# THUDM/CogDL

Measured on NVIDIA B200. Metric: spmm_aggregated_edges_per_sec, higher is better.
Workload: dtype f32

## Files before the change

cogdl_b200/csrc/common.cuh:

```cuda
#pragma once
#include <cuda_runtime.h>
#include <stdint.h>

#include "../../include/cogdl_b200.h"

#if defined(__CUDA_ARCH__) && (__CUDA_ARCH__ < 1000)
#error "libcogdl_b200 is written for sm_100a (B200) only"
#endif

namespace cogdl_b200 {

int set_error(int code, const char *fmt, ...);
void count_launch(int n = 1);
void note_kernel(const char *fmt, ...);
void append_kernel_note(const char *fmt, ...);
int tuning(const char *env_name, int dflt);

#define CB_REQUIRE(cond, ...)                                             \
  do {                                                                    \
    if (!(cond)) return ::cogdl_b200::set_error(COGDL_B200_EINVAL, __VA_ARGS__); \
  } while (0)

#define CB_CUDA(expr)                                                                       \
  do {                                                                                      \
    cudaError_t _e = (expr);                                                                \
    if (_e != cudaSuccess)                                                                  \
      return ::cogdl_b200::set_error(_e == cudaErrorNoKernelImageForDevice ? COGDL_B200_EDEVICE \
                                                                           : COGDL_B200_ECUDA, \
                                     "%s: %s", #expr, cudaGetErrorString(_e));              \
  } while (0)

#define CB_LAUNCH_CHECK()                  \
  do {                                     \
    ::cogdl_b200::count_launch();          \
    CB_CUDA(cudaPeekAtLastError());        \
  } while (0)

static inline bool first_use_on_device(unsigned long long &mask, int *dev) {
  *dev = 0;
  if (cudaGetDevice(dev) != cudaSuccess || *dev < 0 || *dev >= 64) return true;
  const unsigned long long bit = 1ull << *dev;
  if (mask & bit) return false;
  mask |= bit;
  return true;
}

static inline bool aligned16(const void *p) { return (reinterpret_cast<uintptr_t>(p) & 15u) == 0; }
static inline int64_t ceil_div(int64_t a, int64_t b) { return (a + b - 1) / b; }

struct HubView {
  int chunk_edges;
  int n_chunks;
  const int2 *chunks;
  int *counters;
  void *partials;
  int n_segs;
  const int2 *segs;
  const int *edge_row;
  int n_empty_rows;
};

static inline HubView hub_view(const cogdl_b200_hub_plan_t *plan) {
  HubView h{0, 0, nullptr, nullptr, nullptr, 0, nullptr, nullptr, 0};
  if (plan && plan->chunk_edges > 0) {
    h.chunk_edges = plan->chunk_edges;
    h.n_chunks = plan->n_chunks;
    h.chunks = reinterpret_cast<const int2 *>(plan->chunks);
    h.counters = plan->counters;
    h.partials = plan->partials;
    if (plan->segs && plan->edge_row && plan->n_segs > 0) {
      h.n_segs = plan->n_segs;
      h.segs = reinterpret_cast<const int2 *>(plan->segs);
      h.edge_row = plan->edge_row;
      h.n_empty_rows = plan->n_empty_rows;
    }
  }
  return h;
}

int check_plan(const cogdl_b200_hub_plan_t *plan, int64_t need_partial_bytes);

#ifdef __CUDACC__

constexpr unsigned FULL = 0xffffffffu;

__device__ __forceinline__ int ld_stream(const int *p) {
  int v;
  asm volatile("ld.global.nc.L1::no_allocate.s32 %0, [%1];" : "=r"(v) : "l"(p));
  return v;
}
__device__ __forceinline__ float ld_stream(const float *p) {
  float v;
  asm volatile("ld.global.nc.L1::no_allocate.f32 %0, [%1];" : "=f"(v) : "l"(p));
  return v;
}
__device__ __forceinline__ float4 ld_gather(const float4 *p) { return __ldg(p); }
__device__ __forceinline__ float ld_gather(const float *p) { return __ldg(p); }

__device__ __forceinline__ uint64_t l2_policy_evict_last() {
  uint64_t pol;
  asm volatile("createpolicy.fractional.L2::evict_last.b64 %0, 1.0;" : "=l"(pol));
  return pol;
}
__device__ __forceinline__ float4 ld_gather_hint(const float4 *p, uint64_t pol) {
  float4 v;
  asm volatile("ld.global.nc.L2::cache_hint.v4.f32 {%0,%1,%2,%3}, [%4], %5;"
               : "=f"(v.x), "=f"(v.y), "=f"(v.z), "=f"(v.w) : "l"(p), "l"(pol));
  return v;
}
__device__ __forceinline__ float ld_gather_hint(const float *p, uint64_t pol) {
  float v;
  asm volatile("ld.global.nc.L2::cache_hint.f32 %0, [%1], %2;" : "=f"(v) : "l"(p), "l"(pol));
  return v;
}

__device__ __forceinline__ void st_stream(float4 *p, float4 v) { __stcs(p, v); }
__device__ __forceinline__ void st_stream(float *p, float v) { __stcs(p, v); }
__device__ __forceinline__ void st_stream(int *p, int v) { __stcs(p, v); }

__device__ __forceinline__ float4 ld_cg(const float4 *p) { return __ldcg(p); }
__device__ __forceinline__ float ld_cg(const float *p) { return __ldcg(p); }
__device__ __forceinline__ int ld_cg(const int *p) { return __ldcg(p); }
__device__ __forceinline__ void st_cg(float4 *p, float4 v) { __stcg(p, v); }
__device__ __forceinline__ void st_cg(float *p, float v) { __stcg(p, v); }
__device__ __forceinline__ void st_cg(int *p, int v) { __stcg(p, v); }

__device__ __forceinline__ float mul_add_rn(float acc, float v, float x) {
  return __fadd_rn(acc, __fmul_rn(v, x));
}
__device__ __forceinline__ void axpy_rn(float &acc, float v, const float &x) { acc = mul_add_rn(acc, v, x); }
__device__ __forceinline__ void axpy_rn(float4 &acc, float v, const float4 &x) {
  acc.x = mul_add_rn(acc.x, v, x.x);
  acc.y = mul_add_rn(acc.y, v, x.y);
  acc.z = mul_add_rn(acc.z, v, x.z);
  acc.w = mul_add_rn(acc.w, v, x.w);
}
__device__ __forceinline__ void add_rn(float4 &acc, const float4 &x) {
  acc.x = __fadd_rn(acc.x, x.x);
  acc.y = __fadd_rn(acc.y, x.y);
  acc.z = __fadd_rn(acc.z, x.z);
  acc.w = __fadd_rn(acc.w, x.w);
}

template <int WIDTH>
__device__ __forceinline__ int group_max(int v) {
#pragma unroll
  for (int s = WIDTH / 2; s > 0; s >>= 1) v = max(v, __shfl_xor_sync(FULL, v, s));
  return v;
}
__device__ __forceinline__ int warp_max(int v) { return group_max<32>(v); }

struct WorkItem {
  int row;
  int lb, hb;
  int slot;
  int first;
  int n_row_chunks;
  bool active;
  bool is_chunk;
};

__device__ __forceinline__ WorkItem decode_item(int64_t item, int64_t n_rows, const int *__restrict__ rowptr,
                                                const HubView &hub) {
  WorkItem w;
  w.row = 0; w.lb = 0; w.hb = 0; w.slot = 0; w.first = 0; w.n_row_chunks = 0;
  w.active = false; w.is_chunk = false;
  if (item < hub.n_chunks) {
    const int2 c = __ldg(hub.chunks + item);
    const int rb = __ldg(rowptr + c.x), re = __ldg(rowptr + c.x + 1);
    w.row = c.x;
    w.first = c.y;
    w.slot = (int)item;
    w.lb = rb + ((int)item - c.y) * hub.chunk_edges;
    w.hb = min(w.lb + hub.chunk_edges, re);
    w.n_row_chunks = (re - rb + hub.chunk_edges - 1) / hub.chunk_edges;
    w.active = true;
    w.is_chunk = true;
  } else if (item - hub.n_chunks < n_rows) {
    w.row = (int)(item - hub.n_chunks);
    w.lb = __ldg(rowptr + w.row);
    w.hb = __ldg(rowptr + w.row + 1);
    w.active = !(hub.chunk_edges > 0 && (w.hb - w.lb) > hub.chunk_edges);
    if (!w.active) w.hb = w.lb;
  }
  return w;
}

template <int GROUP>
__device__ __forceinline__ bool hub_arrive_last(const WorkItem &w, const HubView &hub, int gl) {
  __threadfence();
  __syncwarp();
  int old = 0;
  if (w.is_chunk && gl == 0) old = atomicAdd(hub.counters + w.first, 1);
  old = __shfl_sync(FULL, old, 0, GROUP);
  const bool last = w.is_chunk && (old == w.n_row_chunks - 1);
  if (last) {
    if (gl == 0) hub.counters[w.first] = 0;
    __threadfence();
  }
  return last;
}

#endif

}
```

cogdl_b200/csrc/spmm.cu:

```cuda
#include "common.cuh"
#include "stream.cuh"

#include <cuda_fp16.h>

#include <cstdlib>

namespace cogdl_b200 {

struct SpmmParams {
  const float *peers[8];
  int n_peers;
  int peer_shift;
  const int *rowptr;
  const int *colind;
  const float *val;
  const float *X0;
  const float *X1;
  int64_t n0;
  float *Y;
  int64_t n_rows;
  int FV;
  HubView hub;
};

template <typename VecT> __device__ __forceinline__ VecT vzero();
template <> __device__ __forceinline__ float4 vzero<float4>() { return make_float4(0.f, 0.f, 0.f, 0.f); }
template <> __device__ __forceinline__ float vzero<float>() { return 0.f; }
__device__ __forceinline__ void add_rn(float &a, const float &b) { a = __fadd_rn(a, b); }

template <typename VecT, int GROUP, int NV, bool HAS_VAL>
__global__ void __launch_bounds__(256) spmm_kernel(const SpmmParams p) {
  constexpr int U0 = (NV == 1) ? 8 : (NV == 2 ? 4 : 2);
  constexpr int U = U0 < GROUP ? U0 : GROUP;
  constexpr int TILE = GROUP * NV;
  const int lane = threadIdx.x & 31;
  const int gl = lane & (GROUP - 1);
  const int64_t tid = (int64_t)blockIdx.x * blockDim.x + threadIdx.x;
  const int64_t item = tid / GROUP;
  const WorkItem w = decode_item(item, p.n_rows, p.rowptr, p.hub);
  const bool warp_has_chunk = (tid - lane) / GROUP < p.hub.n_chunks;

  const VecT *X0 = reinterpret_cast<const VecT *>(p.X0);
  const VecT *X1 = reinterpret_cast<const VecT *>(p.X1);
  VecT *Y = reinterpret_cast<VecT *>(p.Y);
  VecT *P = reinterpret_cast<VecT *>(p.hub.partials);

  int maxdeg = w.hb - w.lb;
  if (GROUP < 32) maxdeg = warp_max(maxdeg);

  for (int tile0 = 0; tile0 < p.FV; tile0 += TILE) {
    const int cv = tile0 + gl;
    bool colok[NV];
#pragma unroll
    for (int k = 0; k < NV; ++k) colok[k] = (cv + k * GROUP) < p.FV;
    VecT acc[NV];
#pragma unroll
    for (int k = 0; k < NV; ++k) acc[k] = vzero<VecT>();

    int c = 0;
    float v = 0.f;
    {
      const int e = w.lb + gl;
      if (e < w.hb) {
        c = ld_stream(p.colind + e);
        v = HAS_VAL ? ld_stream(p.val + e) : 1.f;
      }
    }
    for (int off = 0; off < maxdeg; off += GROUP) {
      const int cnt = min(GROUP, w.hb - w.lb - off);
      int cn = 0;
      float vn = 0.f;
      {
        const int e = w.lb + off + GROUP + gl;
        if (e < w.hb) {
          cn = ld_stream(p.colind + e);
          vn = HAS_VAL ? ld_stream(p.val + e) : 1.f;
        }
      }
#pragma unroll 1
      for (int j = 0; j < GROUP; j += U) {
        if (GROUP == 32) {
          if (j >= cnt) break;
        } else {
          if (!__any_sync(FULL, j < cnt)) break;
        }
        VecT x[U][NV];
#pragma unroll
        for (int u = 0; u < U; ++u) {
          const int cj = __shfl_sync(FULL, c, j + u, GROUP);
          if (j + u < cnt) {
            const VecT *xp = (cj < p.n0) ? X0 + (int64_t)cj * p.FV : X1 + ((int64_t)cj - p.n0) * p.FV;
#pragma unroll
            for (int k = 0; k < NV; ++k)
              if (colok[k]) x[u][k] = ld_gather(xp + cv + k * GROUP);
          }
        }
#pragma unroll
        for (int u = 0; u < U; ++u) {
          const float vj = __shfl_sync(FULL, v, j + u, GROUP);
          if (j + u < cnt) {
#pragma unroll
            for (int k = 0; k < NV; ++k)
              if (colok[k]) axpy_rn(acc[k], vj, x[u][k]);
          }
        }
      }
      c = cn;
      v = vn;
    }

    if (!w.is_chunk) {
      if (w.active) {
        VecT *yp = Y + (int64_t)w.row * p.FV + cv;
#pragma unroll
        for (int k = 0; k < NV; ++k)
          if (colok[k]) st_stream(yp + k * GROUP, acc[k]);
      }
    } else {
      VecT *pp = P + (int64_t)w.slot * p.FV + cv;
#pragma unroll
      for (int k = 0; k < NV; ++k)
        if (colok[k]) st_cg(pp + k * GROUP, acc[k]);
    }
  }

  if (warp_has_chunk) {
    if (hub_arrive_last<GROUP>(w, p.hub, gl)) {
      for (int cv = gl; cv < p.FV; cv += GROUP) {
        const VecT *pp = P + (int64_t)w.first * p.FV + cv;
        VecT s = ld_cg(pp);
        for (int q = 1; q < w.n_row_chunks; ++q) add_rn(s, ld_cg(pp + (int64_t)q * p.FV));
        st_stream(Y + (int64_t)w.row * p.FV + cv, s);
      }
    }
  }
}

static int spmm_variant() { return tuning("COGDL_B200_SPMM_VARIANT", 7); }

static StreamParams to_stream(const SpmmParams &p) {
  StreamParams q;
  q.rowptr = p.rowptr; q.colind = p.colind; q.val = p.val; q.att = nullptr; q.perm = nullptr;
  q.X0 = p.X0; q.X1 = p.X1; q.n0 = p.n0; q.Y = p.Y; q.ldv = p.FV; q.H = 1; q.FVL = p.FV; q.S = 1;
  q.hub = p.hub;
  q.n_peers = p.n_peers; q.peer_shift = p.peer_shift;
  for (int i = 0; i < 8; ++i) q.peers[i] = p.peers[i];
  return q;
}

template <typename VecT, int NV>
static int launch_spmm_stream(const SpmmParams &p, cudaStream_t stream) {
  const StreamParams q = to_stream(p);
  const int mode = p.val ? MODE_WEIGHTED : MODE_UNWEIGHTED;
  if constexpr (NV == 1 && sizeof(VecT) == 16) {
    switch (spmm_variant()) {
      case 1: return launch_stream<VecT, 1, 8, 4, false>(q, mode, stream);
      case 2: return launch_stream<VecT, 1, 8, 3, false>(q, mode, stream);
      case 3: return launch_stream<VecT, 1, 4, 6, false>(q, mode, stream);
      case 8: return launch_stream<VecT, 1, 4, 5, false, true>(q, mode, stream);
      default: return launch_stream<VecT, 1, 4, 5, false>(q, mode, stream);
    }
  }
  constexpr int U = (NV == 1) ? 8 : (NV == 2 ? 4 : 2);
  return launch_stream<VecT, NV, U, 1>(q, mode, stream);
}

template <typename VecT, int GROUP, int NV>
static int launch_spmm(const SpmmParams &p, cudaStream_t stream) {
  const int64_t items = (int64_t)p.hub.n_chunks + p.n_rows;
  const int64_t threads = items * GROUP;
  const int64_t blocks = ceil_div(threads, 256);
  if (blocks == 0) return COGDL_B200_OK;
  if (blocks > 0x7fffffffLL)
    return set_error(COGDL_B200_EINVAL, "spmm: problem too large for one launch (blocks=%lld)", (long long)blocks);
  dim3 grid((unsigned)blocks);
  note_kernel("cogdl_b200::spmm_kernel<%s,GROUP=%d,NV=%d,%s>", sizeof(VecT) == 16 ? "float4" : "float", GROUP, NV,
              p.val ? "weighted" : "unweighted");
  if (p.val)
    spmm_kernel<VecT, GROUP, NV, true><<<grid, 256, 0, stream>>>(p);
  else
    spmm_kernel<VecT, GROUP, NV, false><<<grid, 256, 0, stream>>>(p);
  CB_LAUNCH_CHECK();
  return COGDL_B200_OK;
}

template <typename VecT>
static int dispatch_spmm(const SpmmParams &p, cudaStream_t s) {
  const int fv = p.FV;
  if (p.n_peers > 0 && fv <= 32) return launch_spmm_stream<VecT, 1>(p, s);
  const bool stream = p.hub.n_segs > 0;
  const int stream_min_fv = tuning("COGDL_B200_SPMM_STREAM_MINFV", 9);
  if (stream && fv >= stream_min_fv && fv <= 16) return launch_spmm_stream<VecT, 1>(p, s);
  if (fv <= 1) return launch_spmm<VecT, 1, 1>(p, s);
  if (fv <= 2) return launch_spmm<VecT, 2, 1>(p, s);
  if (fv <= 4) return launch_spmm<VecT, 4, 1>(p, s);
  if (fv <= 8) return launch_spmm<VecT, 8, 1>(p, s);
  if (fv <= 16) return launch_spmm<VecT, 16, 1>(p, s);
  if (fv <= 32) return stream ? launch_spmm_stream<VecT, 1>(p, s) : launch_spmm<VecT, 32, 1>(p, s);
  if (sizeof(VecT) == 4 && fv > 64) return stream ? launch_spmm_stream<VecT, 4>(p, s) : launch_spmm<VecT, 32, 4>(p, s);
  return stream ? launch_spmm_stream<VecT, 2>(p, s) : launch_spmm<VecT, 32, 2>(p, s);
}

static int spmm_entry(const int32_t *rowptr, const int32_t *colind, const float *val, const float *X0,
                      int64_t n0, const float *X1, float *Y, int64_t n_rows, int64_t F,
                      const cogdl_b200_hub_plan_t *plan, cogdl_b200_stream_t stream, const char *who,
                      const float *const *peers = nullptr, int n_peers = 0, int peer_shift = 0) {
  CB_REQUIRE(n_rows >= 0 && F >= 0, "%s: negative size (n_rows=%lld, F=%lld)", who, (long long)n_rows, (long long)F);
  if (n_rows == 0 || F == 0) return COGDL_B200_OK;
  CB_REQUIRE(rowptr && colind && X0 && Y, "%s: null pointer", who);
  CB_REQUIRE(n_rows < 0x7fffffffLL && F < 0x7fffffffLL, "%s: n_rows / F must fit int32", who);
  int rc = check_plan(plan, (plan ? (int64_t)plan->n_chunks : 0) * F * (int64_t)sizeof(float));
  if (rc) return rc;
  SpmmParams p;
  p.rowptr = rowptr; p.colind = colind; p.val = val; p.X0 = X0; p.X1 = X1 ? X1 : X0; p.n0 = n0;
  p.Y = Y; p.n_rows = n_rows; p.hub = hub_view(plan);
  p.n_peers = n_peers; p.peer_shift = peer_shift;
  bool peers_aligned = true;
  for (int i = 0; i < 8; ++i) {
    p.peers[i] = (i < n_peers) ? peers[i] : nullptr;
    peers_aligned = peers_aligned && aligned16(p.peers[i]);
  }
  if (n_peers > 0)
    CB_REQUIRE(p.hub.n_segs > 0 && F % 4 == 0 && F <= 512 && peers_aligned && aligned16(X0) && aligned16(Y),
               "%s: the peer form needs a plan with segments, F %% 4 == 0, F <= 512 and 16-byte aligned buffers", who);
  const bool vec = (F % 4 == 0) && aligned16(X0) && aligned16(p.X1) && aligned16(Y) &&
                   (p.hub.n_chunks == 0 || aligned16(p.hub.partials));
  if (vec) {
    p.FV = (int)(F / 4);
    return dispatch_spmm<float4>(p, (cudaStream_t)stream);
  }
  p.FV = (int)F;
  return dispatch_spmm<float>(p, (cudaStream_t)stream);
}

struct SpmmHalfParams {
  const int *rowptr;
  const int *colind;
  const __half *val;
  const __half *X;
  __half *Y;
  int64_t n_rows;
  int F;
  HubView hub;
};

template <bool HAS_VAL, bool VEC>
__global__ void __launch_bounds__(256) spmm_half_kernel(const SpmmHalfParams p) {
  constexpr int U = 8;
  constexpr int W = VEC ? 4 : 1;
  const int lane = threadIdx.x & 31;
  const int64_t tid = (int64_t)blockIdx.x * blockDim.x + threadIdx.x;
  const WorkItem w = decode_item(tid / 32, p.n_rows, p.rowptr, p.hub);
  float *P = reinterpret_cast<float *>(p.hub.partials);

  for (int tile0 = 0; tile0 < p.F; tile0 += 32 * W) {
    const int col = tile0 + lane * W;
    const bool colok = col < p.F;
    float acc[W];
#pragma unroll
    for (int t = 0; t < W; ++t) acc[t] = 0.f;

    for (int base = w.lb; base < w.hb; base += 32) {
      const int cnt = min(32, w.hb - base);
      int c = 0;
      float v = 0.f;
      if (base + lane < w.hb) {
        c = ld_stream(p.colind + base + lane);
        v = HAS_VAL ? __half2float(p.val[base + lane]) : 1.f;
      }
#pragma unroll 1
      for (int j = 0; j < cnt; j += U) {
        float x[U][W];
#pragma unroll
        for (int u = 0; u < U; ++u) {
          const int cj = __shfl_sync(FULL, c, j + u);
          if (j + u < cnt && colok) {
            const __half *xp = p.X + (int64_t)cj * p.F + col;
            if constexpr (VEC) {
              const uint2 raw = __ldg(reinterpret_cast<const uint2 *>(xp));
              const float2 a = __half22float2(*reinterpret_cast<const __half2 *>(&raw.x));
              const float2 b = __half22float2(*reinterpret_cast<const __half2 *>(&raw.y));
              x[u][0] = a.x; x[u][1] = a.y; x[u][2] = b.x; x[u][3] = b.y;
            } else {
              x[u][0] = __half2float(__ldg(xp));
            }
          }
        }
#pragma unroll
        for (int u = 0; u < U; ++u) {
          const float vj = __shfl_sync(FULL, v, j + u);
          if (j + u < cnt && colok) {
#pragma unroll
            for (int t = 0; t < W; ++t) acc[t] = fmaf(vj, x[u][t], acc[t]);
          }
        }
      }
    }
    if (!w.is_chunk) {
      if (w.active && colok) {
        __half *yp = p.Y + (int64_t)w.row * p.F + col;
#pragma unroll
        for (int t = 0; t < W; ++t) yp[t] = __float2half_rn(acc[t]);
      }
    } else if (colok) {
#pragma unroll
      for (int t = 0; t < W; ++t) st_cg(P + (int64_t)w.slot * p.F + col + t, acc[t]);
    }
  }
  if ((tid - lane) / 32 < p.hub.n_chunks) {
    if (hub_arrive_last<32>(w, p.hub, lane)) {
      for (int col = lane; col < p.F; col += 32) {
        float s = 0.f;
        for (int q = 0; q < w.n_row_chunks; ++q) s += ld_cg(P + (int64_t)(w.first + q) * p.F + col);
        p.Y[(int64_t)w.row * p.F + col] = __float2half_rn(s);
      }
    }
  }
}

int spmm_hub_rows_only(const int32_t *rowptr, const int32_t *colind, const float *val, const float *X, float *Y,
                       int64_t F, const cogdl_b200_hub_plan_t *plan, cudaStream_t stream) {
  SpmmParams p;
  p.rowptr = rowptr; p.colind = colind; p.val = val; p.X0 = X; p.X1 = X; p.n0 = INT64_MAX; p.Y = Y; p.n_rows = 0;
  p.hub = hub_view(plan);
  p.hub.n_segs = 0;
  p.n_peers = 0; p.peer_shift = 0;
  for (int i = 0; i < 8; ++i) p.peers[i] = nullptr;
  p.FV = (int)(F / 4);
  if (p.hub.n_chunks == 0) return COGDL_B200_OK;
  const StreamParams q = to_stream(p);
  if (p.FV <= 32) return launch_stream<float4, 1, 4, 5, false>(q, val ? MODE_WEIGHTED : MODE_UNWEIGHTED, stream);
  return launch_stream<float4, 2, 4, 1>(q, val ? MODE_WEIGHTED : MODE_UNWEIGHTED, stream);
}

}

using namespace cogdl_b200;

extern "C" int cogdl_b200_spmm_csr_f32(const int32_t *rowptr, const int32_t *colind, const float *val,
                                       const float *X, float *Y, int64_t n_rows, int64_t F,
                                       const cogdl_b200_hub_plan_t *plan, cogdl_b200_stream_t stream) {
  return spmm_entry(rowptr, colind, val, X, INT64_MAX, nullptr, Y, n_rows, F, plan, stream,
                    "cogdl_b200_spmm_csr_f32");
}

extern "C" int cogdl_b200_spmm_csr_f32_2src(const int32_t *rowptr, const int32_t *colind, const float *val,
                                            const float *X0, int64_t n0, const float *X1, float *Y,
                                            int64_t n_rows, int64_t F, const cogdl_b200_hub_plan_t *plan,
                                            cogdl_b200_stream_t stream) {
  CB_REQUIRE(n0 >= 0, "cogdl_b200_spmm_csr_f32_2src: n0 < 0");
  CB_REQUIRE(X1 != nullptr || n0 == INT64_MAX, "cogdl_b200_spmm_csr_f32_2src: X1 is null");
  return spmm_entry(rowptr, colind, val, X0, n0, X1, Y, n_rows, F, plan, stream,
                    "cogdl_b200_spmm_csr_f32_2src");
}

extern "C" int cogdl_b200_spmm_csr_f16(const int32_t *rowptr, const int32_t *colind, const void *val,
                                       const void *X, void *Y, int64_t n_rows, int64_t F,
                                       const cogdl_b200_hub_plan_t *plan, cogdl_b200_stream_t stream) {
  CB_REQUIRE(n_rows >= 0 && F >= 0, "cogdl_b200_spmm_csr_f16: negative size");
  if (n_rows == 0 || F == 0) return COGDL_B200_OK;
  CB_REQUIRE(rowptr && colind && X && Y, "cogdl_b200_spmm_csr_f16: null pointer");
  CB_REQUIRE(n_rows < 0x7fffffffLL && F < 0x7fffffffLL, "cogdl_b200_spmm_csr_f16: sizes must fit int32");
  int rc = check_plan(plan, (plan ? (int64_t)plan->n_chunks : 0) * F * (int64_t)sizeof(float));
  if (rc) return rc;
  SpmmHalfParams p;
  p.rowptr = rowptr; p.colind = colind; p.val = (const __half *)val; p.X = (const __half *)X;
  p.Y = (__half *)Y; p.n_rows = n_rows; p.F = (int)F; p.hub = hub_view(plan);
  const bool vec = (F % 4 == 0) && ((reinterpret_cast<uintptr_t>(X) & 7u) == 0);
  const int64_t items = (int64_t)p.hub.n_chunks + n_rows;
  const int64_t blocks = ceil_div(items * 32, 256);
  CB_REQUIRE(blocks <= 0x7fffffffLL, "cogdl_b200_spmm_csr_f16: problem too large");
  dim3 grid((unsigned)blocks);
  cudaStream_t s = (cudaStream_t)stream;
  if (vec) {
    if (val) spmm_half_kernel<true, true><<<grid, 256, 0, s>>>(p);
    else spmm_half_kernel<false, true><<<grid, 256, 0, s>>>(p);
  } else {
    if (val) spmm_half_kernel<true, false><<<grid, 256, 0, s>>>(p);
    else spmm_half_kernel<false, false><<<grid, 256, 0, s>>>(p);
  }
  CB_LAUNCH_CHECK();
  return COGDL_B200_OK;
}

extern "C" int cogdl_b200_spmm_csr_f32_peers(const int32_t *rowptr, const int32_t *colind, const float *val,
                                             const float *X_local, int64_t n_local, const float *const *peer_ptrs,
                                             int32_t n_peers, int32_t owner_shift, float *Y, int64_t n_rows,
                                             int64_t F, const cogdl_b200_hub_plan_t *plan,
                                             cogdl_b200_stream_t stream) {
  CB_REQUIRE(peer_ptrs && n_peers >= 1 && n_peers <= 8, "cogdl_b200_spmm_csr_f32_peers: need 1..8 peer pointers");
  CB_REQUIRE(owner_shift >= 1 && owner_shift <= 28 && n_local >= 0, "cogdl_b200_spmm_csr_f32_peers: bad owner_shift / n_local");
  for (int i = 0; i < n_peers; ++i) CB_REQUIRE(peer_ptrs[i], "cogdl_b200_spmm_csr_f32_peers: null peer pointer %d", i);
  return spmm_entry(rowptr, colind, val, X_local, n_local, nullptr, Y, n_rows, F, plan, stream,
                    "cogdl_b200_spmm_csr_f32_peers", peer_ptrs, n_peers, owner_shift);
}
```

cogdl_b200/csrc/stream.cuh:

```cuda
#pragma once
#include "common.cuh"

namespace cogdl_b200 {

struct StreamParams {
  const int *rowptr;
  const int *colind;
  const float *val;
  const float *att;
  const int *perm;
  const float *X0;
  const float *X1;
  int64_t n0;
  const float *peers[8];
  int n_peers;
  int peer_shift;
  float *Y;
  int ldv;
  int H;
  int FVL;
  int S;
  HubView hub;
};

enum { MODE_UNWEIGHTED = 0, MODE_WEIGHTED = 1, MODE_MULTIHEAD = 2 };
constexpr int STREAM_BLOCK_DEFAULT = 128;
enum { SRC_ONE = 0, SRC_TWO = 1, SRC_PEERS = 2 };

template <typename VecT> __device__ __forceinline__ VecT sk_zero();
template <> __device__ __forceinline__ float4 sk_zero<float4>() { return make_float4(0.f, 0.f, 0.f, 0.f); }
template <> __device__ __forceinline__ float sk_zero<float>() { return 0.f; }
__device__ __forceinline__ void sk_add(float &a, const float &b) { a = __fadd_rn(a, b); }
__device__ __forceinline__ void sk_add(float4 &a, const float4 &b) { add_rn(a, b); }

template <typename VecT, int NV, int MODE, bool HAS_PERM, int SRC, int U, bool ROWS, bool PREFETCH, bool HINT>
__device__ __forceinline__ void stream_range(const StreamParams &p, int e, const int e_end, const int cv,
                                             const bool (&colok)[NV], const int head, const int lane,
                                             VecT (&acc)[NV]) {
  const VecT *X0 = reinterpret_cast<const VecT *>(p.X0) + cv;
  const VecT *X1 = reinterpret_cast<const VecT *>(p.X1) + cv;
  VecT *Y = reinterpret_cast<VecT *>(p.Y) + cv;
  const uint64_t pol = HINT ? l2_policy_evict_last() : 0;

  int c = 0, rid = -1, rnx = -1, pe = 0;
  float v = 0.f;
  auto load_slab = [&](int base, int &c_, float &v_, int &pe_, int &rid_, int &rnx_) {
    const int q = base + lane;
    c_ = 0; v_ = 0.f; pe_ = 0; rid_ = -1; rnx_ = -1;
    if (q < e_end) {
      c_ = ld_stream(p.colind + q);
      if (MODE == MODE_WEIGHTED) v_ = ld_stream(p.val + q);
      if (MODE == MODE_MULTIHEAD) pe_ = HAS_PERM ? ld_stream(p.perm + q) : q;
      if (ROWS) {
        rid_ = ld_stream(p.hub.edge_row + q);
        if (q + 1 < e_end) rnx_ = __ldg(p.hub.edge_row + q + 1);
      }
    }
  };
  load_slab(e, c, v, pe, rid, rnx);

  for (; e < e_end; e += 32) {
    const int cnt = min(32, e_end - e);
    const unsigned endmask = ROWS ? __ballot_sync(FULL, lane < cnt && rid != rnx) : 0u;
    int cn, pn, ridn, rnxn;
    float vn;
    if (PREFETCH) load_slab(e + 32, cn, vn, pn, ridn, rnxn);

#pragma unroll 1
    for (int j = 0; j < cnt; j += U) {
      const bool full = (j + U <= cnt);
      const unsigned em = endmask >> j;
      VecT x[U][NV];
      float a[U];
#pragma unroll
      for (int u = 0; u < U; ++u) {
        const int cj = __shfl_sync(FULL, c, j + u);
        const int pj = (MODE == MODE_MULTIHEAD) ? __shfl_sync(FULL, pe, j + u) : 0;
        if (full || j + u < cnt) {
          const VecT *xp;
          if (SRC == SRC_ONE || cj < p.n0) {
            xp = X0 + (int64_t)cj * p.ldv;
          } else if (SRC == SRC_TWO) {
            xp = X1 + ((int64_t)cj - p.n0) * p.ldv;
          } else {
            const unsigned r = (unsigned)(cj - (int)p.n0);
            xp = reinterpret_cast<const VecT *>(p.peers[r >> p.peer_shift]) + cv +
                 (int64_t)(r & ((1u << p.peer_shift) - 1u)) * p.ldv;
          }
#pragma unroll
          for (int k = 0; k < NV; ++k)
            if (colok[k]) x[u][k] = HINT ? ld_gather_hint(xp + k * 32, pol) : ld_gather(xp + k * 32);
          if (MODE == MODE_MULTIHEAD && colok[0]) a[u] = __ldg(p.att + (int64_t)pj * p.H + head);
        }
      }
#pragma unroll
      for (int u = 0; u < U; ++u) {
        const float vj = (MODE == MODE_WEIGHTED) ? __shfl_sync(FULL, v, j + u) : 0.f;
        const int rj = ROWS ? __shfl_sync(FULL, rid, j + u) : 0;
        if (full || j + u < cnt) {
#pragma unroll
          for (int k = 0; k < NV; ++k) {
            if (colok[k]) {
              if (MODE == MODE_UNWEIGHTED) sk_add(acc[k], x[u][k]);
              else if (MODE == MODE_WEIGHTED) axpy_rn(acc[k], vj, x[u][k]);
              else axpy_rn(acc[k], a[u], x[u][k]);
            }
          }
          if (ROWS && ((em >> u) & 1u)) {
#pragma unroll
            for (int k = 0; k < NV; ++k)
              if (colok[k]) { st_stream(Y + (int64_t)rj * p.ldv + k * 32, acc[k]); acc[k] = sk_zero<VecT>(); }
          }
        }
      }
    }
    if (PREFETCH) { c = cn; v = vn; pe = pn; rid = ridn; rnx = rnxn; }
    else load_slab(e + 32, c, v, pe, rid, rnx);
  }
}

template <typename VecT, int MODE, int SRC, int U, bool ROWS>
__device__ __forceinline__ void stream_range_lean(const StreamParams &p, int e, const int e_end, const int cv, const bool colok,
                                                  const int lane, int2 *s_cv, int *s_r, VecT &acc) {
  const VecT *X0 = reinterpret_cast<const VecT *>(p.X0) + cv;
  const VecT *X1 = reinterpret_cast<const VecT *>(p.X1) + cv;
  VecT *Y = reinterpret_cast<VecT *>(p.Y) + cv;
  auto src_ptr = [&](int cj) -> const VecT * {
    if (SRC == SRC_ONE || cj < p.n0) return X0 + (int64_t)cj * p.ldv;
    if (SRC == SRC_TWO) return X1 + ((int64_t)cj - p.n0) * p.ldv;
    const unsigned r = (unsigned)(cj - (int)p.n0);
    return reinterpret_cast<const VecT *>(p.peers[r >> p.peer_shift]) + cv + (int64_t)(r & ((1u << p.peer_shift) - 1u)) * p.ldv;
  };
  auto accumulate = [&](float vj, const VecT &x) {
    if (MODE == MODE_UNWEIGHTED) sk_add(acc, x); else axpy_rn(acc, vj, x);
  };
  for (; e < e_end; e += 32) {
    const int cnt = min(32, e_end - e);
    const int q = e + lane;
    int c = 0, rid = -1, rnx = -1;
    float v = 0.f;
    if (q < e_end) {
      c = ld_stream(p.colind + q);
      if (MODE == MODE_WEIGHTED) v = ld_stream(p.val + q);
      if (ROWS) {
        rid = ld_stream(p.hub.edge_row + q);
        if (q + 1 < e_end) rnx = __ldg(p.hub.edge_row + q + 1);
      }
    }
    const unsigned endmask = ROWS ? __ballot_sync(FULL, lane < cnt && rid != rnx) : 0u;
    __syncwarp();
    s_cv[lane] = make_int2(c, __float_as_int(v));
    if (ROWS) s_r[lane] = rid;
    __syncwarp();
    int j = 0;
#pragma unroll 1
    for (; j + U <= cnt; j += U) {
      int2 cw[U];
      VecT x[U];
#pragma unroll
      for (int u = 0; u < U; ++u) cw[u] = s_cv[j + u];
#pragma unroll
      for (int u = 0; u < U; ++u)
        if (colok) x[u] = ld_gather(src_ptr(cw[u].x));
      const unsigned em = ROWS ? ((endmask >> j) & ((1u << U) - 1u)) : 0u;
      if (em == 0u) {
#pragma unroll
        for (int u = 0; u < U; ++u)
          if (colok) accumulate(__int_as_float(cw[u].y), x[u]);
      } else {
#pragma unroll
        for (int u = 0; u < U; ++u) {
          if (colok) accumulate(__int_as_float(cw[u].y), x[u]);
          if ((em >> u) & 1u) {
            const int rj = s_r[j + u];
            if (colok) { st_stream(Y + (int64_t)rj * p.ldv, acc); acc = sk_zero<VecT>(); }
          }
        }
      }
    }
#pragma unroll 1
    for (; j < cnt; ++j) {
      const int2 cw = s_cv[j];
      if (colok) accumulate(__int_as_float(cw.y), ld_gather(src_ptr(cw.x)));
      if (ROWS && ((endmask >> j) & 1u)) {
        const int rj = s_r[j];
        if (colok) { st_stream(Y + (int64_t)rj * p.ldv, acc); acc = sk_zero<VecT>(); }
      }
    }
  }
}

template <typename VecT, int NV, int MODE, bool HAS_PERM, int SRC, int U, bool PREFETCH, bool HINT>
__device__ __forceinline__ void stream_item(const StreamParams &p, const int64_t wid, const int lane, int2 *s_cv, int *s_r) {
  constexpr int TILE = 32 * NV;
  const int64_t item = (MODE == MODE_MULTIHEAD) ? wid / p.S : wid;
  const int slice = (MODE == MODE_MULTIHEAD) ? (int)(wid - item * p.S) : 0;
  VecT *Y = reinterpret_cast<VecT *>(p.Y);
  VecT *P = reinterpret_cast<VecT *>(p.hub.partials);
  constexpr bool LEAN = (NV == 1 && MODE != MODE_MULTIHEAD && !HINT);

  const int t_begin = (MODE == MODE_MULTIHEAD) ? slice * 32 : 0;
  const int t_end = (MODE == MODE_MULTIHEAD) ? t_begin + 1 : p.ldv;

  if (item < p.hub.n_chunks) {
    const WorkItem w = decode_item(item, 0, p.rowptr, p.hub);
    for (int tile0 = t_begin; tile0 < t_end; tile0 += TILE) {
      const int cv = tile0 + lane;
      bool colok[NV];
      VecT acc[NV];
#pragma unroll
      for (int k = 0; k < NV; ++k) { colok[k] = (cv + k * 32) < p.ldv; acc[k] = sk_zero<VecT>(); }
      const int head = (MODE == MODE_MULTIHEAD && colok[0]) ? cv / p.FVL : 0;
      if constexpr (LEAN) stream_range_lean<VecT, MODE, SRC, U, false>(p, w.lb, w.hb, cv, colok[0], lane, s_cv, s_r, acc[0]);
      else stream_range<VecT, NV, MODE, HAS_PERM, SRC, U, false, PREFETCH, HINT>(p, w.lb, w.hb, cv, colok, head, lane, acc);
#pragma unroll
      for (int k = 0; k < NV; ++k)
        if (colok[k]) st_cg(P + (int64_t)w.slot * p.ldv + cv + k * 32, acc[k]);
    }
    WorkItem wa = w;
    wa.n_row_chunks = w.n_row_chunks * p.S;
    if (hub_arrive_last<32>(wa, p.hub, lane)) {
      for (int cv = lane; cv < p.ldv; cv += 32) {
        const VecT *pp = P + (int64_t)w.first * p.ldv + cv;
        VecT s = ld_cg(pp);
        int q = 1;
        for (; q + 8 <= w.n_row_chunks; q += 8) {
          VecT t[8];
#pragma unroll
          for (int u = 0; u < 8; ++u) t[u] = ld_cg(pp + (int64_t)(q + u) * p.ldv);
#pragma unroll
          for (int u = 0; u < 8; ++u) sk_add(s, t[u]);
        }
        for (; q < w.n_row_chunks; ++q) sk_add(s, ld_cg(pp + (int64_t)q * p.ldv));
        st_stream(Y + (int64_t)w.row * p.ldv + cv, s);
      }
    }
    return;
  }

  const int64_t seg = item - p.hub.n_chunks;
  if (seg >= p.hub.n_segs) return;
  const int2 rr = __ldg(p.hub.segs + seg);
  const int e_begin = __ldg(p.rowptr + rr.x), e_end = __ldg(p.rowptr + rr.y);

  for (int tile0 = t_begin; tile0 < t_end; tile0 += TILE) {
    const int cv = tile0 + lane;
    bool colok[NV];
    VecT acc[NV];
#pragma unroll
    for (int k = 0; k < NV; ++k) { colok[k] = (cv + k * 32) < p.ldv; acc[k] = sk_zero<VecT>(); }
    const int head = (MODE == MODE_MULTIHEAD && colok[0]) ? cv / p.FVL : 0;
    if (p.hub.n_empty_rows > 0) {
      for (int rb = rr.x; rb < rr.y; rb += 32) {
        const int row = rb + lane;
        unsigned m = __ballot_sync(FULL, row < rr.y && __ldg(p.rowptr + row + 1) == __ldg(p.rowptr + row));
        while (m) {
          const int k0 = __ffs(m) - 1;
          m &= m - 1;
#pragma unroll
          for (int k = 0; k < NV; ++k)
            if (colok[k]) st_stream(Y + (int64_t)(rb + k0) * p.ldv + cv + k * 32, sk_zero<VecT>());
        }
      }
    }
    if constexpr (LEAN) stream_range_lean<VecT, MODE, SRC, U, true>(p, e_begin, e_end, cv, colok[0], lane, s_cv, s_r, acc[0]);
    else stream_range<VecT, NV, MODE, HAS_PERM, SRC, U, true, PREFETCH, HINT>(p, e_begin, e_end, cv, colok, head, lane, acc);
  }
}

template <typename VecT, int NV, int MODE, bool HAS_PERM, int SRC, int U, int MINB, bool PREFETCH, bool HINT>
__global__ void __launch_bounds__(256, MINB) stream_kernel(const StreamParams p) {
  const int lane = threadIdx.x & 31;
  constexpr bool LEAN = (NV == 1 && MODE != MODE_MULTIHEAD && !HINT);
  __shared__ int2 s_cv_all[LEAN ? 8 : 1][32];
  __shared__ int s_r_all[LEAN ? 8 : 1][32];
  int2 *s_cv = s_cv_all[LEAN ? (threadIdx.x >> 5) : 0];
  int *s_r = s_r_all[LEAN ? (threadIdx.x >> 5) : 0];
  const int64_t wid = ((int64_t)blockIdx.x * blockDim.x + threadIdx.x) >> 5;
  stream_item<VecT, NV, MODE, HAS_PERM, SRC, U, PREFETCH, HINT>(p, wid, lane, s_cv, s_r);
}

template <typename VecT, int NV, int U, int MINB, bool PREFETCH = true, bool HINT = false>
static int launch_stream(const StreamParams &p, int mode, cudaStream_t stream) {
  const int64_t warps = ((int64_t)p.hub.n_chunks + p.hub.n_segs) * p.S;
  int bs = tuning("COGDL_B200_STREAM_BLOCK", STREAM_BLOCK_DEFAULT);
  if (bs != 32 && bs != 64 && bs != 128) bs = 256;
  const int64_t blocks = ceil_div(warps * 32, bs);
  if (blocks == 0) return COGDL_B200_OK;
  if (blocks > 0x7fffffffLL) return set_error(COGDL_B200_EINVAL, "stream kernel: problem too large for one launch");
  const unsigned g = (unsigned)blocks;
  const int src = p.n_peers > 0 ? SRC_PEERS : (p.n0 != INT64_MAX ? SRC_TWO : SRC_ONE);
  note_kernel("cogdl_b200::stream_kernel<%s,NV=%d,%s%s,%s,U=%d,MINB=%d%s%s>", sizeof(VecT) == 16 ? "float4" : "float", NV,
              mode == MODE_MULTIHEAD ? "multihead" : (mode == MODE_WEIGHTED ? "weighted" : "unweighted"),
              (mode == MODE_MULTIHEAD && p.perm) ? "+perm" : "",
              src == SRC_PEERS ? "SRC_PEERS" : (src == SRC_TWO ? "SRC_TWO" : "SRC_ONE"), U, MINB,
              PREFETCH ? ",prefetch" : "", HINT ? ",l2hint" : "");
  if (bs != 256) append_kernel_note(" block=%d", bs);
  if (mode == MODE_MULTIHEAD) {
    if constexpr (NV == 1) {
      if (p.perm) stream_kernel<VecT, 1, MODE_MULTIHEAD, true, SRC_ONE, U, MINB, PREFETCH, HINT><<<g, bs, 0, stream>>>(p);
      else stream_kernel<VecT, 1, MODE_MULTIHEAD, false, SRC_ONE, U, MINB, PREFETCH, HINT><<<g, bs, 0, stream>>>(p);
    } else {
      return set_error(COGDL_B200_EINVAL, "stream kernel: multi-head form needs NV == 1");
    }
  } else if (mode == MODE_WEIGHTED) {
    if (src == SRC_PEERS) stream_kernel<VecT, NV, MODE_WEIGHTED, false, SRC_PEERS, U, MINB, PREFETCH, HINT><<<g, bs, 0, stream>>>(p);
    else if (src == SRC_TWO) stream_kernel<VecT, NV, MODE_WEIGHTED, false, SRC_TWO, U, MINB, PREFETCH, HINT><<<g, bs, 0, stream>>>(p);
    else stream_kernel<VecT, NV, MODE_WEIGHTED, false, SRC_ONE, U, MINB, PREFETCH, HINT><<<g, bs, 0, stream>>>(p);
  } else {
    if (src == SRC_PEERS) stream_kernel<VecT, NV, MODE_UNWEIGHTED, false, SRC_PEERS, U, MINB, PREFETCH, HINT><<<g, bs, 0, stream>>>(p);
    else if (src == SRC_TWO) stream_kernel<VecT, NV, MODE_UNWEIGHTED, false, SRC_TWO, U, MINB, PREFETCH, HINT><<<g, bs, 0, stream>>>(p);
    else stream_kernel<VecT, NV, MODE_UNWEIGHTED, false, SRC_ONE, U, MINB, PREFETCH, HINT><<<g, bs, 0, stream>>>(p);
  }
  CB_LAUNCH_CHECK();
  return COGDL_B200_OK;
}

}
```

Baseline: 14.15 billion.

## Replace lean stream loop with cp.async shared-memory ring pipeline for gathers

The lean per-warp stream loop used for NV==1 SpMM is replaced by a cp.async-based pipeline. It double-buffers column, value and row-id slabs and keeps a ring of R gathered X rows in shared memory, so several batches of gathers are in flight ahead of the accumulation. The kernel moves to dynamic shared memory sized per warp, and the default variant switches to a 12-deep ring with MINB=4. The L2 evict_last hint path is removed. In exchange it uses more shared memory, which can lower occupancy, and adds wait/commit overhead and extra bookkeeping for tails and row ends.

```diff
diff --git a/cogdl_b200/csrc/common.cuh b/cogdl_b200/csrc/common.cuh
--- a/cogdl_b200/csrc/common.cuh
+++ b/cogdl_b200/csrc/common.cuh
@@ -97,22 +97,21 @@
 __device__ __forceinline__ float4 ld_gather(const float4 *p) { return __ldg(p); }
 __device__ __forceinline__ float ld_gather(const float *p) { return __ldg(p); }
 
-__device__ __forceinline__ uint64_t l2_policy_evict_last() {
-  uint64_t pol;
-  asm volatile("createpolicy.fractional.L2::evict_last.b64 %0, 1.0;" : "=l"(pol));
-  return pol;
-}
-__device__ __forceinline__ float4 ld_gather_hint(const float4 *p, uint64_t pol) {
-  float4 v;
-  asm volatile("ld.global.nc.L2::cache_hint.v4.f32 {%0,%1,%2,%3}, [%4], %5;"
-               : "=f"(v.x), "=f"(v.y), "=f"(v.z), "=f"(v.w) : "l"(p), "l"(pol));
-  return v;
-}
-__device__ __forceinline__ float ld_gather_hint(const float *p, uint64_t pol) {
-  float v;
-  asm volatile("ld.global.nc.L2::cache_hint.f32 %0, [%1], %2;" : "=f"(v) : "l"(p), "l"(pol));
-  return v;
-}
+__device__ __forceinline__ void cp_async(float4 *dst, const float4 *src) {
+  asm volatile("cp.async.cg.shared.global [%0], [%1], 16;" ::"r"((unsigned)__cvta_generic_to_shared(dst)), "l"(src)
+               : "memory");
+}
+__device__ __forceinline__ void cp_async(float *dst, const float *src) {
+  asm volatile("cp.async.ca.shared.global [%0], [%1], 4;" ::"r"((unsigned)__cvta_generic_to_shared(dst)), "l"(src)
+               : "memory");
+}
+__device__ __forceinline__ void cp_async(int *dst, const int *src) {
+  asm volatile("cp.async.ca.shared.global [%0], [%1], 4;" ::"r"((unsigned)__cvta_generic_to_shared(dst)), "l"(src)
+               : "memory");
+}
+__device__ __forceinline__ void cp_async_commit() { asm volatile("cp.async.commit_group;" ::: "memory"); }
+template <int N>
+__device__ __forceinline__ void cp_async_wait() { asm volatile("cp.async.wait_group %0;" ::"n"(N) : "memory"); }
 
 __device__ __forceinline__ void st_stream(float4 *p, float4 v) { __stcs(p, v); }
 __device__ __forceinline__ void st_stream(float *p, float v) { __stcs(p, v); }
diff --git a/cogdl_b200/csrc/spmm.cu b/cogdl_b200/csrc/spmm.cu
--- a/cogdl_b200/csrc/spmm.cu
+++ b/cogdl_b200/csrc/spmm.cu
@@ -136,7 +136,7 @@
   }
 }
 
-static int spmm_variant() { return tuning("COGDL_B200_SPMM_VARIANT", 7); }
+static int spmm_variant() { return tuning("COGDL_B200_SPMM_VARIANT", 2); }
 
 static StreamParams to_stream(const SpmmParams &p) {
   StreamParams q;
@@ -148,21 +148,25 @@
   return q;
 }
 
+template <typename VecT>
+static int launch_spmm_ring(const StreamParams &q, int mode, cudaStream_t stream) {
+  switch (spmm_variant()) {
+    case 1: return launch_stream<VecT, 1, 4, 5, false, 8>(q, mode, stream);
+    case 3: return launch_stream<VecT, 1, 4, 3, false, 16>(q, mode, stream);
+    default: return launch_stream<VecT, 1, 4, 4, false, 12>(q, mode, stream);
+  }
+}
+
 template <typename VecT, int NV>
 static int launch_spmm_stream(const SpmmParams &p, cudaStream_t stream) {
   const StreamParams q = to_stream(p);
   const int mode = p.val ? MODE_WEIGHTED : MODE_UNWEIGHTED;
-  if constexpr (NV == 1 && sizeof(VecT) == 16) {
-    switch (spmm_variant()) {
-      case 1: return launch_stream<VecT, 1, 8, 4, false>(q, mode, stream);
-      case 2: return launch_stream<VecT, 1, 8, 3, false>(q, mode, stream);
-      case 3: return launch_stream<VecT, 1, 4, 6, false>(q, mode, stream);
-      case 8: return launch_stream<VecT, 1, 4, 5, false, true>(q, mode, stream);
-      default: return launch_stream<VecT, 1, 4, 5, false>(q, mode, stream);
-    }
-  }
-  constexpr int U = (NV == 1) ? 8 : (NV == 2 ? 4 : 2);
-  return launch_stream<VecT, NV, U, 1>(q, mode, stream);
+  if constexpr (NV == 1) {
+    return launch_spmm_ring<VecT>(q, mode, stream);
+  } else {
+    constexpr int U = (NV == 2) ? 4 : 2;
+    return launch_stream<VecT, NV, U, 1>(q, mode, stream);
+  }
 }
 
 template <typename VecT, int GROUP, int NV>
@@ -329,7 +333,7 @@
   p.FV = (int)(F / 4);
   if (p.hub.n_chunks == 0) return COGDL_B200_OK;
   const StreamParams q = to_stream(p);
-  if (p.FV <= 32) return launch_stream<float4, 1, 4, 5, false>(q, val ? MODE_WEIGHTED : MODE_UNWEIGHTED, stream);
+  if (p.FV <= 32) return launch_spmm_ring<float4>(q, val ? MODE_WEIGHTED : MODE_UNWEIGHTED, stream);
   return launch_stream<float4, 2, 4, 1>(q, val ? MODE_WEIGHTED : MODE_UNWEIGHTED, stream);
 }
 
diff --git a/cogdl_b200/csrc/stream.cuh b/cogdl_b200/csrc/stream.cuh
--- a/cogdl_b200/csrc/stream.cuh
+++ b/cogdl_b200/csrc/stream.cuh
@@ -1,4 +1,6 @@
 #pragma once
+#include <cstdio>
+
 #include "common.cuh"
 
 namespace cogdl_b200 {
@@ -33,14 +35,13 @@
 __device__ __forceinline__ void sk_add(float &a, const float &b) { a = __fadd_rn(a, b); }
 __device__ __forceinline__ void sk_add(float4 &a, const float4 &b) { add_rn(a, b); }
 
-template <typename VecT, int NV, int MODE, bool HAS_PERM, int SRC, int U, bool ROWS, bool PREFETCH, bool HINT>
+template <typename VecT, int NV, int MODE, bool HAS_PERM, int SRC, int U, bool ROWS, bool PREFETCH>
 __device__ __forceinline__ void stream_range(const StreamParams &p, int e, const int e_end, const int cv,
                                              const bool (&colok)[NV], const int head, const int lane,
                                              VecT (&acc)[NV]) {
   const VecT *X0 = reinterpret_cast<const VecT *>(p.X0) + cv;
   const VecT *X1 = reinterpret_cast<const VecT *>(p.X1) + cv;
   VecT *Y = reinterpret_cast<VecT *>(p.Y) + cv;
-  const uint64_t pol = HINT ? l2_policy_evict_last() : 0;
 
   int c = 0, rid = -1, rnx = -1, pe = 0;
   float v = 0.f;
@@ -89,7 +90,7 @@
           }
 #pragma unroll
           for (int k = 0; k < NV; ++k)
-            if (colok[k]) x[u][k] = HINT ? ld_gather_hint(xp + k * 32, pol) : ld_gather(xp + k * 32);
+            if (colok[k]) x[u][k] = ld_gather(xp + k * 32);
           if (MODE == MODE_MULTIHEAD && colok[0]) a[u] = __ldg(p.att + (int64_t)pj * p.H + head);
         }
       }
@@ -119,9 +120,23 @@
   }
 }
 
-template <typename VecT, int MODE, int SRC, int U, bool ROWS>
-__device__ __forceinline__ void stream_range_lean(const StreamParams &p, int e, const int e_end, const int cv, const bool colok,
-                                                  const int lane, int2 *s_cv, int *s_r, VecT &acc) {
+template <typename VecT, int R>
+struct RingSmem {
+  VecT ring[R > 0 ? R : 1][32];
+  int2 cv[2][32];
+  int r[2][33];
+};
+
+template <typename VecT, int MODE, int SRC, int U, int R, bool ROWS>
+__device__ __forceinline__ void stream_range_ring(const StreamParams &p, const int e, const int e_end, const int cv,
+                                                  const bool colok, const int lane, RingSmem<VecT, R> &s, VecT &acc) {
+  constexpr int D = R / U;
+  constexpr int BPS = 32 / U;
+  static_assert(R % U == 0 && 32 % U == 0 && D >= 1 && 2 * D <= BPS, "ring: R must be a multiple of U and <= 16");
+  const int n = e_end - e;
+  if (n <= 0) return;
+  const int nb = (n + U - 1) / U;
+  const int nslab = (n + 31) >> 5;
   const VecT *X0 = reinterpret_cast<const VecT *>(p.X0) + cv;
   const VecT *X1 = reinterpret_cast<const VecT *>(p.X1) + cv;
   VecT *Y = reinterpret_cast<VecT *>(p.Y) + cv;
@@ -134,70 +149,91 @@
   auto accumulate = [&](float vj, const VecT &x) {
     if (MODE == MODE_UNWEIGHTED) sk_add(acc, x); else axpy_rn(acc, vj, x);
   };
-  for (; e < e_end; e += 32) {
-    const int cnt = min(32, e_end - e);
-    const int q = e + lane;
-    int c = 0, rid = -1, rnx = -1;
-    float v = 0.f;
+  auto issue_slab = [&](int k) {
+    const int q = e + (k << 5) + lane;
     if (q < e_end) {
-      c = ld_stream(p.colind + q);
-      if (MODE == MODE_WEIGHTED) v = ld_stream(p.val + q);
-      if (ROWS) {
-        rid = ld_stream(p.hub.edge_row + q);
-        if (q + 1 < e_end) rnx = __ldg(p.hub.edge_row + q + 1);
-      }
-    }
-    const unsigned endmask = ROWS ? __ballot_sync(FULL, lane < cnt && rid != rnx) : 0u;
-    __syncwarp();
-    s_cv[lane] = make_int2(c, __float_as_int(v));
-    if (ROWS) s_r[lane] = rid;
-    __syncwarp();
-    int j = 0;
+      cp_async(&s.cv[k & 1][lane].x, p.colind + q);
+      if (MODE == MODE_WEIGHTED) cp_async(reinterpret_cast<float *>(&s.cv[k & 1][lane].y), p.val + q);
+      if (ROWS) cp_async(&s.r[k & 1][lane], p.hub.edge_row + q);
+    }
+    if (ROWS && lane == 31 && q + 1 < e_end) cp_async(&s.r[k & 1][32], p.hub.edge_row + q + 1);
+  };
+  auto slab_endmask = [&](int k) -> unsigned {
+    const int q = e + (k << 5) + lane;
+    const int *rb = s.r[k & 1];
+    return __ballot_sync(FULL, q < e_end && (q == e_end - 1 || rb[lane] != rb[lane + 1]));
+  };
+  auto issue_batch = [&](int b, int slot) {
+    if (b >= nb || !colok) return;
+    const int2 *cw = s.cv[(b / BPS) & 1] + (b % BPS) * U;
+#pragma unroll
+    for (int u = 0; u < U; ++u)
+      if (b * U + u < n) cp_async(&s.ring[slot * U + u][lane], src_ptr(cw[u].x));
+  };
+
+  __syncwarp();
+  issue_slab(0);
+  cp_async_commit();
+  cp_async_wait<0>();
+  __syncwarp();
+  unsigned em_cur = ROWS ? slab_endmask(0) : 0u, em_next = 0u;
+  if (nslab > 1) issue_slab(1);
+#pragma unroll
+  for (int d = 0; d < D; ++d) {
+    issue_batch(d, d);
+    cp_async_commit();
+  }
+  int slot = 0;
 #pragma unroll 1
-    for (; j + U <= cnt; j += U) {
-      int2 cw[U];
-      VecT x[U];
-#pragma unroll
-      for (int u = 0; u < U; ++u) cw[u] = s_cv[j + u];
-#pragma unroll
-      for (int u = 0; u < U; ++u)
-        if (colok) x[u] = ld_gather(src_ptr(cw[u].x));
-      const unsigned em = ROWS ? ((endmask >> j) & ((1u << U) - 1u)) : 0u;
-      if (em == 0u) {
+  for (int k = 0; k < nslab; ++k) {
+    if (k > 0) {
+      __syncwarp();
+      if (k + 1 < nslab) issue_slab(k + 1);
+      em_cur = em_next;
+    }
+#pragma unroll 1
+    for (int j = 0; j < BPS; ++j) {
+      const int b = k * BPS + j;
+      if (b >= nb) break;
+      cp_async_wait<D - 1>();
+      if (j == BPS - D && k + 1 < nslab) {
+        __syncwarp();
+        if (ROWS) em_next = slab_endmask(k + 1);
+      }
+      const int2 *cw = s.cv[k & 1] + j * U;
+      const unsigned em = ROWS ? ((em_cur >> (j * U)) & ((1u << U) - 1u)) : 0u;
+      const bool full = (b + 1) * U <= n;
+      if (full && em == 0u) {
 #pragma unroll
         for (int u = 0; u < U; ++u)
-          if (colok) accumulate(__int_as_float(cw[u].y), x[u]);
+          if (colok) accumulate(__int_as_float(cw[u].y), s.ring[slot * U + u][lane]);
       } else {
 #pragma unroll
         for (int u = 0; u < U; ++u) {
-          if (colok) accumulate(__int_as_float(cw[u].y), x[u]);
+          if (!full && b * U + u >= n) break;
+          if (colok) accumulate(__int_as_float(cw[u].y), s.ring[slot * U + u][lane]);
           if ((em >> u) & 1u) {
-            const int rj = s_r[j + u];
+            const int rj = s.r[k & 1][j * U + u];
             if (colok) { st_stream(Y + (int64_t)rj * p.ldv, acc); acc = sk_zero<VecT>(); }
           }
         }
       }
-    }
-#pragma unroll 1
-    for (; j < cnt; ++j) {
-      const int2 cw = s_cv[j];
-      if (colok) accumulate(__int_as_float(cw.y), ld_gather(src_ptr(cw.x)));
-      if (ROWS && ((endmask >> j) & 1u)) {
-        const int rj = s_r[j];
-        if (colok) { st_stream(Y + (int64_t)rj * p.ldv, acc); acc = sk_zero<VecT>(); }
-      }
-    }
-  }
-}
-
-template <typename VecT, int NV, int MODE, bool HAS_PERM, int SRC, int U, bool PREFETCH, bool HINT>
-__device__ __forceinline__ void stream_item(const StreamParams &p, const int64_t wid, const int lane, int2 *s_cv, int *s_r) {
+      issue_batch(b + D, slot);
+      cp_async_commit();
+      slot = (slot + 1 == D) ? 0 : slot + 1;
+    }
+  }
+}
+
+template <typename VecT, int NV, int MODE, bool HAS_PERM, int SRC, int U, bool PREFETCH, int R>
+__device__ __forceinline__ void stream_item(const StreamParams &p, const int64_t wid, const int lane, RingSmem<VecT, R> &s) {
   constexpr int TILE = 32 * NV;
   const int64_t item = (MODE == MODE_MULTIHEAD) ? wid / p.S : wid;
   const int slice = (MODE == MODE_MULTIHEAD) ? (int)(wid - item * p.S) : 0;
   VecT *Y = reinterpret_cast<VecT *>(p.Y);
   VecT *P = reinterpret_cast<VecT *>(p.hub.partials);
-  constexpr bool LEAN = (NV == 1 && MODE != MODE_MULTIHEAD && !HINT);
+  constexpr bool RING = (R > 0);
+  static_assert(!RING || (NV == 1 && MODE != MODE_MULTIHEAD), "the ring loop serves the plain SpMM with NV == 1");
 
   const int t_begin = (MODE == MODE_MULTIHEAD) ? slice * 32 : 0;
   const int t_end = (MODE == MODE_MULTIHEAD) ? t_begin + 1 : p.ldv;
@@ -211,8 +247,8 @@
 #pragma unroll
       for (int k = 0; k < NV; ++k) { colok[k] = (cv + k * 32) < p.ldv; acc[k] = sk_zero<VecT>(); }
       const int head = (MODE == MODE_MULTIHEAD && colok[0]) ? cv / p.FVL : 0;
-      if constexpr (LEAN) stream_range_lean<VecT, MODE, SRC, U, false>(p, w.lb, w.hb, cv, colok[0], lane, s_cv, s_r, acc[0]);
-      else stream_range<VecT, NV, MODE, HAS_PERM, SRC, U, false, PREFETCH, HINT>(p, w.lb, w.hb, cv, colok, head, lane, acc);
+      if constexpr (RING) stream_range_ring<VecT, MODE, SRC, U, R, false>(p, w.lb, w.hb, cv, colok[0], lane, s, acc[0]);
+      else stream_range<VecT, NV, MODE, HAS_PERM, SRC, U, false, PREFETCH>(p, w.lb, w.hb, cv, colok, head, lane, acc);
 #pragma unroll
       for (int k = 0; k < NV; ++k)
         if (colok[k]) st_cg(P + (int64_t)w.slot * p.ldv + cv + k * 32, acc[k]);
@@ -263,24 +299,38 @@
         }
       }
     }
-    if constexpr (LEAN) stream_range_lean<VecT, MODE, SRC, U, true>(p, e_begin, e_end, cv, colok[0], lane, s_cv, s_r, acc[0]);
-    else stream_range<VecT, NV, MODE, HAS_PERM, SRC, U, true, PREFETCH, HINT>(p, e_begin, e_end, cv, colok, head, lane, acc);
-  }
-}
-
-template <typename VecT, int NV, int MODE, bool HAS_PERM, int SRC, int U, int MINB, bool PREFETCH, bool HINT>
+    if constexpr (RING) stream_range_ring<VecT, MODE, SRC, U, R, true>(p, e_begin, e_end, cv, colok[0], lane, s, acc[0]);
+    else stream_range<VecT, NV, MODE, HAS_PERM, SRC, U, true, PREFETCH>(p, e_begin, e_end, cv, colok, head, lane, acc);
+  }
+}
+
+template <typename VecT, int NV, int MODE, bool HAS_PERM, int SRC, int U, int MINB, bool PREFETCH, int R>
 __global__ void __launch_bounds__(256, MINB) stream_kernel(const StreamParams p) {
+  extern __shared__ __align__(16) unsigned char s_dyn[];
   const int lane = threadIdx.x & 31;
-  constexpr bool LEAN = (NV == 1 && MODE != MODE_MULTIHEAD && !HINT);
-  __shared__ int2 s_cv_all[LEAN ? 8 : 1][32];
-  __shared__ int s_r_all[LEAN ? 8 : 1][32];
-  int2 *s_cv = s_cv_all[LEAN ? (threadIdx.x >> 5) : 0];
-  int *s_r = s_r_all[LEAN ? (threadIdx.x >> 5) : 0];
+  RingSmem<VecT, R> *s = reinterpret_cast<RingSmem<VecT, R> *>(s_dyn) + (R > 0 ? (threadIdx.x >> 5) : 0);
   const int64_t wid = ((int64_t)blockIdx.x * blockDim.x + threadIdx.x) >> 5;
-  stream_item<VecT, NV, MODE, HAS_PERM, SRC, U, PREFETCH, HINT>(p, wid, lane, s_cv, s_r);
-}
-
-template <typename VecT, int NV, int U, int MINB, bool PREFETCH = true, bool HINT = false>
+  stream_item<VecT, NV, MODE, HAS_PERM, SRC, U, PREFETCH, R>(p, wid, lane, *s);
+}
+
+template <typename VecT, int NV, int MODE, bool HAS_PERM, int SRC, int U, int MINB, bool PREFETCH, int R>
+static int launch_stream_kernel(const StreamParams &p, unsigned g, int bs, cudaStream_t stream) {
+  auto kernel = stream_kernel<VecT, NV, MODE, HAS_PERM, SRC, U, MINB, PREFETCH, R>;
+  size_t smem = 0;
+  if constexpr (R > 0) {
+    constexpr int per_warp = (int)sizeof(RingSmem<VecT, R>);
+    static unsigned long long attr_done = 0;
+    int dev = 0;
+    if (first_use_on_device(attr_done, &dev))
+      CB_CUDA(cudaFuncSetAttribute(kernel, cudaFuncAttributeMaxDynamicSharedMemorySize, 8 * per_warp));
+    smem = (size_t)(bs / 32) * per_warp;
+  }
+  kernel<<<g, bs, smem, stream>>>(p);
+  CB_LAUNCH_CHECK();
+  return COGDL_B200_OK;
+}
+
+template <typename VecT, int NV, int U, int MINB, bool PREFETCH = true, int R = 0>
 static int launch_stream(const StreamParams &p, int mode, cudaStream_t stream) {
   const int64_t warps = ((int64_t)p.hub.n_chunks + p.hub.n_segs) * p.S;
   int bs = tuning("COGDL_B200_STREAM_BLOCK", STREAM_BLOCK_DEFAULT);
@@ -290,30 +340,29 @@
   if (blocks > 0x7fffffffLL) return set_error(COGDL_B200_EINVAL, "stream kernel: problem too large for one launch");
   const unsigned g = (unsigned)blocks;
   const int src = p.n_peers > 0 ? SRC_PEERS : (p.n0 != INT64_MAX ? SRC_TWO : SRC_ONE);
-  note_kernel("cogdl_b200::stream_kernel<%s,NV=%d,%s%s,%s,U=%d,MINB=%d%s%s>", sizeof(VecT) == 16 ? "float4" : "float", NV,
+  char ring[16] = "";
+  if (R > 0) snprintf(ring, sizeof(ring), ",R=%d", R);
+  note_kernel("cogdl_b200::stream_kernel<%s,NV=%d,%s%s,%s,U=%d%s,MINB=%d%s>", sizeof(VecT) == 16 ? "float4" : "float", NV,
               mode == MODE_MULTIHEAD ? "multihead" : (mode == MODE_WEIGHTED ? "weighted" : "unweighted"),
               (mode == MODE_MULTIHEAD && p.perm) ? "+perm" : "",
-              src == SRC_PEERS ? "SRC_PEERS" : (src == SRC_TWO ? "SRC_TWO" : "SRC_ONE"), U, MINB,
-              PREFETCH ? ",prefetch" : "", HINT ? ",l2hint" : "");
+              src == SRC_PEERS ? "SRC_PEERS" : (src == SRC_TWO ? "SRC_TWO" : "SRC_ONE"), U, ring, MINB,
+              PREFETCH ? ",prefetch" : "");
   if (bs != 256) append_kernel_note(" block=%d", bs);
   if (mode == MODE_MULTIHEAD) {
-    if constexpr (NV == 1) {
-      if (p.perm) stream_kernel<VecT, 1, MODE_MULTIHEAD, true, SRC_ONE, U, MINB, PREFETCH, HINT><<<g, bs, 0, stream>>>(p);
-      else stream_kernel<VecT, 1, MODE_MULTIHEAD, false, SRC_ONE, U, MINB, PREFETCH, HINT><<<g, bs, 0, stream>>>(p);
+    if constexpr (NV == 1 && R == 0) {
+      if (p.perm) return launch_stream_kernel<VecT, 1, MODE_MULTIHEAD, true, SRC_ONE, U, MINB, PREFETCH, R>(p, g, bs, stream);
+      return launch_stream_kernel<VecT, 1, MODE_MULTIHEAD, false, SRC_ONE, U, MINB, PREFETCH, R>(p, g, bs, stream);
     } else {
-      return set_error(COGDL_B200_EINVAL, "stream kernel: multi-head form needs NV == 1");
+      return set_error(COGDL_B200_EINVAL, "stream kernel: multi-head form needs NV == 1 and no ring");
     }
   } else if (mode == MODE_WEIGHTED) {
-    if (src == SRC_PEERS) stream_kernel<VecT, NV, MODE_WEIGHTED, false, SRC_PEERS, U, MINB, PREFETCH, HINT><<<g, bs, 0, stream>>>(p);
-    else if (src == SRC_TWO) stream_kernel<VecT, NV, MODE_WEIGHTED, false, SRC_TWO, U, MINB, PREFETCH, HINT><<<g, bs, 0, stream>>>(p);
-    else stream_kernel<VecT, NV, MODE_WEIGHTED, false, SRC_ONE, U, MINB, PREFETCH, HINT><<<g, bs, 0, stream>>>(p);
-  } else {
-    if (src == SRC_PEERS) stream_kernel<VecT, NV, MODE_UNWEIGHTED, false, SRC_PEERS, U, MINB, PREFETCH, HINT><<<g, bs, 0, stream>>>(p);
-    else if (src == SRC_TWO) stream_kernel<VecT, NV, MODE_UNWEIGHTED, false, SRC_TWO, U, MINB, PREFETCH, HINT><<<g, bs, 0, stream>>>(p);
-    else stream_kernel<VecT, NV, MODE_UNWEIGHTED, false, SRC_ONE, U, MINB, PREFETCH, HINT><<<g, bs, 0, stream>>>(p);
-  }
-  CB_LAUNCH_CHECK();
-  return COGDL_B200_OK;
-}
-
-}
+    if (src == SRC_PEERS) return launch_stream_kernel<VecT, NV, MODE_WEIGHTED, false, SRC_PEERS, U, MINB, PREFETCH, R>(p, g, bs, stream);
+    if (src == SRC_TWO) return launch_stream_kernel<VecT, NV, MODE_WEIGHTED, false, SRC_TWO, U, MINB, PREFETCH, R>(p, g, bs, stream);
+    return launch_stream_kernel<VecT, NV, MODE_WEIGHTED, false, SRC_ONE, U, MINB, PREFETCH, R>(p, g, bs, stream);
+  }
+  if (src == SRC_PEERS) return launch_stream_kernel<VecT, NV, MODE_UNWEIGHTED, false, SRC_PEERS, U, MINB, PREFETCH, R>(p, g, bs, stream);
+  if (src == SRC_TWO) return launch_stream_kernel<VecT, NV, MODE_UNWEIGHTED, false, SRC_TWO, U, MINB, PREFETCH, R>(p, g, bs, stream);
+  return launch_stream_kernel<VecT, NV, MODE_UNWEIGHTED, false, SRC_ONE, U, MINB, PREFETCH, R>(p, g, bs, stream);
+}
+
+}
```

Result: slower. 13.47 billion (median of 6 runs) (-4.8%).
